# jirsat/wavenets

Measured on AMD Instinct MI355X. Metric: audio samples/sec (training step, 16 kHz mu-law), higher is better.
Workload: dtype f32 (fp16 hi|lo split operands, fp32 accumulate)

## Files before the change

### wavenets_amd/csrc/wn_kernels.h

```cpp
#pragma once
#include "wn_common.h"

struct WnTensorDesc { int64_t off; int64_t len; };

struct WnPrepDesc {
  int64_t src_off;
  int64_t dst_off;
  int32_t I;
  int32_t KK;
  int32_t ld;
  int32_t transpose;
  int32_t q_off;
  int32_t j_off;
  int32_t JT;
  int32_t kind;
};
int wn_launch_prep_table(const WnPrepDesc* d_table, int n, const float* params, float* ws,
                         hipStream_t s, int gx = 16);
int wn_launch_prep_one(WnPrepDesc d, const float* params, float* ws, hipStream_t s);
struct WnVecSumArgs { const float* base; int64_t off0; int64_t stride; int32_t count; int32_t len; float* out; };
int wn_launch_vecsum(WnVecSumArgs a, hipStream_t s);

#define WN_MAXSEG 4
struct WnSeg {
// ... 44 lines not shown
  int32_t act;
  float* y; int32_t ldy;
  int32_t N;
  int32_t B, T;
  float* absmax_out;
  int32_t bwd;
  const float* absmax_in;
  const float* aux; int32_t ld_aux;
  int32_t nshift; int32_t shift[4];
  int32_t cat_loss;
  const int32_t* target;
  float gscale;
  float* loss_rows;
  float* sample_out;
  float inv_lv;
  uint64_t seed, offset;
};
int wn_gemm_planes16s_supported(int N, int plane_k, int nplanes, int ld, int ldy);
int wn_gemm_taps16s_supported(int N, int plane_k, int ntaps, int ld, int ldy);
int wn_launch_gemm_planes16s(const WnGemmPlanesArgs& a, hipStream_t s);

struct WnWgradArgs {
  const float* x; int32_t ldx; int32_t K; int32_t shift;
  const float* g; int32_t ldg; int32_t N;
  int32_t B, T;
  int32_t splits_per_b;
  float* slab;
  float* slab_bias;
};
int wn_wgrad_choose_splits(int B, int T, int K, int N);
int wn_launch_wgrad(const WnWgradArgs& a, hipStream_t s);
struct WnWgJob {
  int64_t x_off, g_off, out_off, bias_off;
  int64_t gmax_off;
  int32_t ldx, ldg, K, N, shift, k0, n0, pad_;
};
struct WnWgLayer {
  int64_t x_off, du_off, z_off, go_off;
  int64_t dwd_off, dbd_off, dwr_off, dbr_off;
  int64_t gmax_u_off, gmax_h_off;
  int32_t dilation, ldz;
};
int wn_wgrad_layer_supported(int R, int D, int KS);
int wn_launch_wgrad_layers(const WnWgLayer* d_layers, int nlayers, int R, float* ws, float* slab, int64_t P, int B,
                           int T, int splits_per_b, hipStream_t s, int inner = 0);
struct WnWgPair {
  int64_t x_off, g_off;
  int64_t w_off, b_off;
  int64_t gmax_off;
  int32_t shift;
  union { int32_t pad_; int32_t nseg; };
  union { int64_t g2_off; int64_t seg_stride; };
  int64_t w2_off, b2_off, gmax2_off;
};
int wn_wgrad_pair_kind(int K, int N);
int wn_launch_wgrad_pairs(int kind, const WnWgPair* d_jobs, int njobs, float* ws, float* slab, int64_t P, int B, int T,
                          int splits_per_b, hipStream_t s);
int wn_wgrad_tr_kind(int K, int N, int taps);
int wn_launch_wgrad_tr(int kind, const WnWgPair* d_jobs, int njobs, float* ws, float* slab, int64_t P, int B, int T,
                       int splits_per_b, hipStream_t s, float* slab2 = nullptr, int64_t P2 = 0);
struct WnBwdPairArgs {
  const float* gu_in;
  const float* gx_res;
  const float* gf;
  const float* ag;
  const float* z; int32_t ldz;
  float* gx_out;
  float* gu_out;
  const float* wx16;
  const float* wu16;
  const float* am_gu_in; const float* am_gf;
  float* am_gx; float* am_gu;
  int32_t B, T, dil;
};
int wn_bwd_pair_supported(int R, int D, int KS, int F0);
int wn_launch_bwd_pair(const WnBwdPairArgs& a, hipStream_t s);
int wn_bwd_s128_supported(int R, int D, int KS, int F0);
int wn_launch_bwd_s128(const WnBwdPairArgs& a, hipStream_t s);
int wn_wgrad_skip_supported(int D, int S, int KZ);
int wn_launch_wgrad_skip(const float* z, int ldz, const float* g, int ldg, int64_t rows, int KZ, int S, int D,
                         int nsplit, float* slab, int64_t P, int64_t w_off0, int64_t w_stride, int64_t b_off0,
                         int64_t b_stride, int nblocks, const float* gmax, hipStream_t s);
int wn_wgrad_tile_k();
int wn_wgrad_tile_n();
int wn_launch_wgrad_batched(const WnWgJob* d_jobs, int njobs, float* ws, float* slab, int64_t P, int B, int T,
                            int splits_per_b, hipStream_t s, bool exact_fp32 = false);
int wn_launch_reduce_table(const float* slab, int nsplit, int64_t P, float* out, const WnTensorDesc* d_table,
                           int n, hipStream_t s, const WnTensorDesc* h_table = nullptr);
struct WnReduceArgs {
  const float* slab; int32_t nsplit; int32_t K; int32_t N;
  float* out; int32_t seg_len; int64_t seg_stride; int32_t accumulate;
  int32_t replicate; int64_t rep_stride;
};
int wn_launch_reduce(const WnReduceArgs& a, hipStream_t s);

struct WnLayerFwdArgs {
  const float* x;
  const float* frag_d;
  const float* frag_r;
  const float* bias_d;
  const float* bias_r;
  const float* cb;
  float* x_out;
  float* o_out;
  float* z_out; int32_t ldz;
  float* ag_out;
// ... 174 lines not shown
```

### wavenets_amd/csrc/wn_train.hip

```cpp
#include "wn_plan_internal.h"

namespace {
using namespace wnp;

void add_jobs(std::vector<WnWgJob>& jobs, int64_t x_off, int ldx, int K, int shift, int64_t g_off, int ldg, int N,
              int64_t out_off, int64_t bias_off, int64_t gmax_off) {
  const int tk = wn_wgrad_tile_k(), tn = wn_wgrad_tile_n();
  for (int k0 = 0; k0 < K; k0 += tk)
    for (int n0 = 0; n0 < N; n0 += tn) {
      WnWgJob j;
      memset(&j, 0, sizeof(j));
      j.x_off = x_off; j.g_off = g_off; j.out_off = out_off; j.bias_off = (k0 == 0) ? bias_off : -1;
      j.gmax_off = gmax_off;
      j.ldx = ldx; j.ldg = ldg; j.K = K; j.N = N; j.shift = shift; j.k0 = k0; j.n0 = n0;
      jobs.push_back(j);
    }
}

int ensure_schedule(const wn_plan* p, wn_exec& e, const WsLayout& L, int B, int T, const TrainPaths& tp) {
  WgSchedule& g = e.wg;
  if (g.valid && g.B == B && g.T == T && g.bsplits == L.bsplits && g.paths == tp) return WN_OK;
  const bool layerk = tp.layerk(), pairk = tp.pairk(), fold = tp.fold;
  std::vector<WnWgLayer> wgl, wgli;
  std::vector<WnWgPair> pairs[3];
// ... 38 lines not shown
      w.dwd_off = p->tensors[c.kernel_t].off; w.dbd_off = p->tensors[c.bias_t].off;
      w.dwr_off = p->tensors[bi.conv1.kernel_t].off; w.dbr_off = p->tensors[bi.conv1.bias_t].off;
      w.gmax_u_off = am_GU(b); w.gmax_h_off = p->S == 0 ? am_skip : am_GH(b + 1);
      w.dilation = c.dil;
      wgl.push_back(w);
    } else if (pairk) {
      const int64_t xoff = tp.drop ? L.XD[b] : L.H[b];
      {
        WnWgPair w;
        memset(&w, 0, sizeof(w));
        w.x_off = xoff; w.g_off = L.GU[b]; w.shift = c.dil;
        w.w_off = p->tensors[c.kernel_t].off;
        w.b_off = p->tensors[c.bias_t].off;
        w.gmax_off = am_GU(b);
        pairs[1].push_back(w);
      }
      WnWgPair w;
      memset(&w, 0, sizeof(w));
      w.x_off = zoff; w.g_off = p->S == 0 ? L.GO[b] : L.GH[b + 1]; w.shift = 0;
      w.w_off = p->tensors[bi.conv1.kernel_t].off; w.b_off = p->tensors[bi.conv1.bias_t].off;
      w.gmax_off = p->S == 0 ? am_skip : am_GH(b + 1);
      w.g2_off = w.w2_off = w.b2_off = w.gmax2_off = -1;
      if (tp.mfused) {
        w.g2_off = L.GF[0]; w.w2_off = (int64_t)b * p->D * p->fold_F0;
        w.b2_off = b == 0 ? (int64_t)p->N * p->D * p->fold_F0 : -1;
        w.gmax2_off = L.absmax + slot.gf(0);
      }
      pairs[2].push_back(w);
    } else {
    for (int i = 0; i < p->LPB; ++i) {
      const ConvInfo& ci = bi.dil[i];
      const bool lastc = i == p->LPB - 1;
      const int64_t xo = i == 0 ? (tp.drop ? L.XD[b] : L.H[b]) : L.P[b][i - 1];
      const int kc = i == 0 ? p->R : p->D, nc = lastc ? 2 * p->D : p->D;
      for (int t = 0; t < p->KS; ++t)
        add_jobs(jobs, xo, kc, kc, (p->KS - 1 - t) * ci.dil, lastc ? L.GU[b] : L.GP[b][i], nc, nc,
                 p->tensors[ci.kernel_t].off + (int64_t)t * kc * nc,
                 t == p->KS - 1 ? p->tensors[ci.bias_t].off : -1, lastc ? am_GU(b) : am_GP(b, i));
      if (!lastc) { cover(ci.kernel_t); cover(ci.bias_t); }
    }
    add_jobs(jobs, zoff, p->Dp, p->D, 0, p->S == 0 ? L.GO[b] : L.GH[b + 1], p->R, p->R,
             p->tensors[bi.conv1.kernel_t].off, p->tensors[bi.conv1.bias_t].off, p->S == 0 ? am_skip : am_GH(b + 1));
    }
    cover(bi.dil.back().kernel_t); cover(bi.dil.back().bias_t);
    cover(bi.conv1.kernel_t); cover(bi.conv1.bias_t);
    if (bi.has_skip && p->c.use_skip && !fold) {
      if (!tp.skipk)
        add_jobs(jobs, zoff, p->Dp, p->D, 0, L.g_skipsum, p->S, p->S,
                 p->tensors[bi.conv_skip.kernel_t].off, p->tensors[bi.conv_skip.bias_t].off, am_skip);
      cover(bi.conv_skip.kernel_t); cover(bi.conv_skip.bias_t);
    }
  }
  if (tp.mtr != 0) {
    const int per = 256 / p->D;
    for (int b0 = 0; b0 < p->N; b0 += per) {
      WnWgPair w;
      memset(&w, 0, sizeof(w));
      w.x_off = L.Z + (int64_t)b0 * B * T * p->Dp;
      w.seg_stride = (int64_t)B * T * p->Dp;
      w.nseg = std::min(per, p->N - b0);
      w.g_off = L.GF[0]; w.shift = 0;
      w.w_off = (int64_t)b0 * p->D * p->fold_F0;
      w.b_off = b0 == 0 ? (int64_t)p->N * p->D * p->fold_F0 : -1;
      w.gmax_off = L.absmax + slot.gf(0);
      w.w2_off = w.b2_off = w.gmax2_off = -1;
      pairs[0].push_back(w);
    }
  }
  const int head_first = (int)jobs.size(), cov_head = (int)cov.size();
  for (size_t i = fold ? 1 : 0; i < p->finals.size(); ++i) {
    const ConvInfo& c = p->finals[i];
    const int64_t xin = (i == 0) ? (p->c.use_skip ? L.skipsum : L.H[p->N]) : L.HA[i - 1];
    if (tp.headpairs() && wn_wgrad_pair_kind(c.cin, c.cout) != 0) {
      WnWgPair w;
      memset(&w, 0, sizeof(w));
      w.x_off = xin; w.g_off = L.GF[i]; w.shift = 0;
      w.w_off = p->tensors[c.kernel_t].off; w.b_off = p->tensors[c.bias_t].off;
      w.gmax_off = L.absmax + slot.gf((int)i);
      const int kind = wn_wgrad_pair_kind(c.cin, c.cout);
      hpairs[kind].push_back(w);
      if (kind == 5) {
        w.g_off += 128; w.w_off += 128; w.b_off += 128;
        hpairs[kind].push_back(w);
      }
    } else {
      add_jobs(jobs, xin, c.cin, c.cin, 0, L.GF[i], c.cout, c.cout, p->tensors[c.kernel_t].off,
               p->tensors[c.bias_t].off, L.absmax + slot.gf((int)i));
    }
    cover(c.kernel_t); cover(c.bias_t);
  }
  std::vector<WnWgPair> all;
  int pfirst[3], hfirst[6] = {0, 0, 0, 0, 0, 0};
  for (int kd = 0; kd <= 2; ++kd) { pfirst[kd] = (int)all.size(); all.insert(all.end(), pairs[kd].begin(), pairs[kd].end()); }
  for (int kd = 1; kd <= 5; ++kd) { hfirst[kd] = (int)all.size(); all.insert(all.end(), hpairs[kd].begin(), hpairs[kd].end()); }
  std::vector<WgSpan> spans;
  auto span = [&](WgSpan::Op op, WgSpan::Slab slab, int kind, int first, size_t count) {
    if (count > 0) spans.push_back(WgSpan{op, slab, kind, first, (int)count});
  };
  const int njobs = (int)jobs.size();
  const bool head_own = tp.head_split && (head_first < njobs || tp.headpairs());
  span(WgSpan::INCONV, WgSpan::BATCH, 0, 0, tp.in_split);
  span(WgSpan::JOBS, WgSpan::BATCH, tp.wg == WG_GENERIC_FP32, 0, head_own ? head_first : njobs);
  if (head_own) span(WgSpan::JOBS, WgSpan::HEAD, 0, head_first, njobs - head_first);
  for (int kd = 1; kd <= 5; ++kd) {
    const int trk = kd == 1 ? 3 : (kd == 3 ? 4 : (kd == 5 ? 5 : (kd == 2 ? 2 : 0)));
    if (trk != 0 && tp.pairk()) span(WgSpan::TR, WgSpan::HEAD, trk, hfirst[kd], hpairs[kd].size());
    else span(WgSpan::PAIRS, WgSpan::HEAD, kd, hfirst[kd], hpairs[kd].size());
  }
  const int n_side = (int)spans.size();
  span(WgSpan::TR, WgSpan::BATCH, 1, pfirst[1], pairs[1].size());
  span(WgSpan::TR, WgSpan::BATCH, tp.mfused ? 6 : 2, pfirst[2], pairs[2].size());
  span(WgSpan::LAYERS, WgSpan::BATCH, 0, 0, wgl.size());
  span(WgSpan::LAYERS, WgSpan::BATCH, 1, 0, wgli.size());
  if (tp.mtr != 0) span(WgSpan::TR, WgSpan::MFOLD, tp.mtr, pfirst[0], pairs[0].size());
  else if (tp.fold) span(WgSpan::SKIP, WgSpan::MFOLD, 0, 0, !tp.mfused);
  else span(WgSpan::SKIP, WgSpan::BATCH, 0, 0, tp.skipk);
  g.valid = false;
  int rc = g.jobs.upload(jobs, 1);
  if (!rc) rc = g.cov.upload(cov);
  if (!rc) rc = g.layers.upload(wgl);
  if (!rc) rc = g.inner.upload(wgli);
  if (!rc) rc = g.pairs.upload(all);
  if (rc) return rc;
  g.h_cov.swap(cov); g.spans.swap(spans);
  g.n_side = n_side; g.overlap = layerk || pairk; g.cov_head = head_own ? cov_head : (int)g.h_cov.size();
  g.B = B; g.T = T; g.bsplits = L.bsplits; g.paths = tp;
  g.valid = true;
  return WN_OK;
}

struct TrainCall {
  wn_exec& e;
  wn_plan* p; const float* params; const float* x_full; const float* cond;
  int B, T, global_batch, n_replicas;
  float* grads; float* loss_out; float* pred_out; float* ws; hipStream_t s;
  WsLayout L;
  int64_t rows;
  float* inputs;
  const float* fragbase; float* slab;
  float* am; AbsmaxSlots slot;
  int nf; float* am_gskip;
  const float* mlast = nullptr;
  TrainPaths tp;
  bool cond_batched = false;
  float* g_x = nullptr; float* g_cond = nullptr;
  int64_t pm = 0;
  float* am_GF(int i) const { return am + slot.gf(i); }
  float* am_GU(int b) const { return am + slot.gu(b); }
  float* am_GH(int b) const { return am + slot.gh(b); }
  float* am_GP(int b, int i) const { return am + slot.gp(b, i); }
  struct Strided { int64_t off, stride; };
  Strided strided(int t0, int t1) const { return {p->tensors[t0].off, p->N > 1 ? p->tensors[t1].off - p->tensors[t0].off : 0}; }
  Strided skip_w{0, 0}, skip_b{0, 0};

  void bind(wn_plan* p_, const float* params_, const float* cond_, int B_, int T_, float* grads_, float* workspace, hipStream_t s_) {
    p = p_; params = params_; x_full = nullptr; cond = cond_; B = B_; T = T_; global_batch = B_; n_replicas = 1;
    grads = grads_; loss_out = nullptr; pred_out = nullptr; ws = workspace; s = s_;
    L = make_layout(p, B, T, true);
    rows = (int64_t)B * T;
    inputs = workspace + L.probs;
    am = workspace + L.absmax;
    nf = (int)p->finals.size();
    slot = AbsmaxSlots{nf, p->N, p->LPB};
    am_gskip = am + slot.gskip();
  }
// ... 185 lines not shown
    rc = wn_launch_sgemm_small(ws + L.mtot, F0, 1, wf0, 1, F0, ws + L.ytmp, p->S, nd1, p->S, F0, s);
    if (rc) return rc;
    const int nzk = (nd1 + 127) / 128;
    if ((int64_t)nzk * p->S * F0 <= L.slab_floats) {
      rc = wn_launch_sgemm_small_batched(ws + L.wsall, 1, p->S, (int64_t)128 * p->S, ws + L.mtot, F0, 1, (int64_t)128 * F0, slab, F0,
                                         (int64_t)p->S * F0, p->S, F0, nd1, nzk, nullptr, 0, s, 128);
      if (rc) return rc;
      WnVecSumArgs v;
      v.base = slab; v.off0 = 0; v.stride = (int64_t)p->S * F0; v.count = nzk; v.len = p->S * F0;
      v.out = grads + p->tensors[c0.kernel_t].off;
      rc = wn_launch_vecsum(v, s);
    } else
    rc = wgrad(ws + L.wsall, p->S, p->S, 0, ws + L.mtot, F0, F0, 1, nd1, grads + p->tensors[c0.kernel_t].off, nullptr, nullptr,
               slab, s);
    if (rc) return rc;
    return wn_launch_skip_scatter(ws + L.ytmp, ws + L.mtot + (int64_t)p->N * p->D * F0, skip_w.off, skip_w.stride, skip_b.off,
                                  skip_b.stride, p->tensors[c0.bias_t].off, p->N, p->D, p->S, F0, grads, s);
  }

  int cond_weight_gradients() {
    int rc;
    const int D2 = 2 * p->D;
    const BlockInfo& b0 = p->blocks[0]; const BlockInfo& b1 = p->blocks[p->N > 1 ? 1 : 0];
    const Strided db = strided(b0.dil.back().bias_t, b1.dil.back().bias_t);
    const Strided cw = strided(b0.conv_cond.kernel_t, b1.conv_cond.kernel_t), cbi = strided(b0.conv_cond.bias_t, b1.conv_cond.bias_t);
    rc = wn_launch_cond_gather(ws + L.bslab, p->nparams, L.bsplits, db.off, db.stride, B, p->N, D2, ws + L.cbt, s);
    if (rc) return rc;
    if (cond_small(p) && (int64_t)p->N * B * p->Cc <= L.slab_floats) {
      rc = wn_launch_sgemm_small_batched(ws + L.cbt, p->N * D2, 1, D2, params + cw.off, 1, D2, cw.stride,
                                         slab, p->Cc, (int64_t)B * p->Cc, B, p->Cc, D2, p->N, nullptr, 0, s);
      if (rc) return rc;
      WnVecSumArgs v;
      v.base = slab; v.off0 = 0; v.stride = (int64_t)B * p->Cc; v.count = p->N; v.len = B * p->Cc; v.out = ws + L.g_m0;
      rc = wn_launch_vecsum(v, s);
    } else
    rc = Gemm(1, B, p->Cc, ceil32(p->Cc)).seg(ws + L.cbt, p->N * D2, p->N * D2, 0, fragbase + p->frag_condB).run(ws + L.g_m0, p->Cc, s);
    if (rc) return rc;
    return wn_launch_cond_wgrad(mlast, ws + L.cbt, B, p->Cc, p->N, D2, grads, cw.off, cw.stride, cbi.off, cbi.stride, s);
  }

  int launch(const WgSpan& sp, hipStream_t st) {
    const WgSchedule& g = e.wg;
    float* out = ws + L.bslab; int64_t pitch = p->nparams; int splits = L.bsplits;
    if (sp.slab == WgSpan::HEAD) { out = ws + L.hslab - L.head_base; pitch = L.head_span; splits = L.hsplits; }
    if (sp.slab == WgSpan::MFOLD) { out = ws + L.mslab; pitch = pm; }
    switch (sp.op) {
      case WgSpan::INCONV:
        return wn_launch_inconv_wgrad(inputs, ws + L.GH[0], B, T, p->R, p->KS, L.isplits, ws + L.islab, (int64_t)(p->KS + 1) * p->R,
                                      0, (int64_t)p->KS * p->R, st);
      case WgSpan::JOBS: return wn_launch_wgrad_batched(g.jobs.d + sp.first, sp.count, ws, out, pitch, B, T, splits, st, sp.kind != 0);
      case WgSpan::PAIRS: return wn_launch_wgrad_pairs(sp.kind, g.pairs.d + sp.first, sp.count, ws, out, pitch, B, T, splits, st);
      case WgSpan::TR:
        return wn_launch_wgrad_tr(sp.kind, g.pairs.d + sp.first, sp.count, ws, out, pitch, B, T, splits, st,
                                  sp.kind == 6 ? ws + L.mslab : nullptr, sp.kind == 6 ? pm : 0);
      case WgSpan::LAYERS: return wn_launch_wgrad_layers(sp.kind ? g.inner.d : g.layers.d, sp.count, p->R, ws, out, pitch, B, T, splits, st, sp.kind);
      case WgSpan::SKIP:
        if (sp.slab == WgSpan::MFOLD)
          return wn_launch_wgrad_skip(ws + L.Z, p->Dp, ws + L.GF[0], p->fold_F0, rows, p->N * p->D, p->fold_F0, p->D, B * splits, out, pitch,
                                      0, (int64_t)p->D * p->fold_F0, (int64_t)p->N * p->D * p->fold_F0, 0, 1, am_GF(0), st);
        return wn_launch_wgrad_skip(ws + L.Z, p->Dp, ws + L.g_skipsum, p->S, rows, p->N * p->D, p->S, p->D, B * splits, out, pitch,
                                    skip_w.off, skip_w.stride, skip_b.off, skip_b.stride, p->N, am_gskip, st);
    }
    return WN_E_INVALID;
  }

  int weight_gradients() {
    int rc;
    const WgSchedule& g = e.wg;
    if (e.phase_on) (void)hipEventRecord(e.phase_ev[3], s);
    const bool fork = g.overlap && wn_debug_get(9) != 1;
    if (fork && !e.side) {
      WN_HIP_CHECK(hipStreamCreateWithFlags(&e.side, hipStreamNonBlocking));
      WN_HIP_CHECK(hipEventCreateWithFlags(&e.ev_fork, hipEventDisableTiming));
      WN_HIP_CHECK(hipEventCreateWithFlags(&e.ev_join, hipEventDisableTiming));
    }
    struct SideJoin {
      wn_exec& e; hipStream_t s; bool armed;
      ~SideJoin() {
        if (!armed) return;
        if (hipEventRecord(e.ev_join, e.side) != hipSuccess || hipStreamWaitEvent(s, e.ev_join, 0) != hipSuccess)
          (void)hipStreamSynchronize(e.side);
      }
    } side_join{e, s, false};
    if (fork) {
      WN_HIP_CHECK(hipEventRecord(e.ev_fork, s));
      WN_HIP_CHECK(hipStreamWaitEvent(e.side, e.ev_fork, 0));
      side_join.armed = true;
    }
    size_t i = 0;
    for (; i < (size_t)g.n_side; ++i)
      if ((rc = launch(g.spans[i], fork ? e.side : s))) return rc;
    if (fork) WN_HIP_CHECK(hipEventRecord(e.ev_join, e.side));
    for (; i < g.spans.size(); ++i)
      if ((rc = launch(g.spans[i], s))) return rc;
    if (tp.fold && (rc = fold_weight_gradients())) return rc;
    if (fork) { WN_HIP_CHECK(hipStreamWaitEvent(s, e.ev_join, 0)); side_join.armed = false; }
    if (cond_batched && (rc = cond_weight_gradients())) return rc;
    const int cov0 = tp.in_split ? 2 : 0, ncov = (int)g.h_cov.size(), cov1 = g.cov_head;
    rc = wn_launch_reduce_table(ws + L.bslab, B * L.bsplits, p->nparams, grads, g.cov.d + cov0, cov1 - cov0, s, g.h_cov.data() + cov0);
    if (rc) return rc;
    if (tp.in_split && (rc = wn_launch_reduce_table(ws + L.islab, B * L.isplits, (int64_t)(p->KS + 1) * p->R, grads, g.cov.d, 2, s, g.h_cov.data())))
      return rc;
    if (cov1 < ncov && (rc = wn_launch_reduce_table(ws + L.hslab - L.head_base, B * L.hsplits, L.head_span, grads, g.cov.d + cov1, ncov - cov1,
                                                    s, g.h_cov.data() + cov1)))
      return rc;
    if (!p->c.use_skip && p->S > 0) {
      for (const BlockInfo& bi : p->blocks) {
        rc = wn_launch_fill(grads + p->tensors[bi.conv_skip.kernel_t].off, 0.f, p->tensors[bi.conv_skip.kernel_t].len, s);
// ... 195 lines not shown
```

### wavenets_amd/csrc/wn_wgrad_layer.hip

```cpp
#include "wn_split16.h"

using namespace wn_split16;

template <int C32, bool INNER>
__global__ __launch_bounds__(256, 2) void wn_wgrad_layer_kernel(const WnWgLayer* layers, float* ws, float* slab,
                                                                int64_t P, int B, int T, int spb) {
  constexpr int R = 32 * C32, NCH = INNER ? 3 * R : 6 * R;
  constexpr int DUW = INNER ? R : 2 * R;
  constexpr int NXU = INNER ? 2 * 2 * R : 2 * 4 * R;
  constexpr int NU = 1 + (NXU + 255) / 256;
  constexpr int PLANE = NCH * 32;
  constexpr int STAGE = 2 * PLANE;
  constexpr int NJ = INNER ? C32 : ((C32 == 2) ? 4 : 1);
  __shared__ __attribute__((aligned(16))) unsigned char smem[2 * STAGE + 2 * NCH * 4];
  float* bpart = reinterpret_cast<float*>(smem + 2 * STAGE);
  const int tid = threadIdx.x, lane = tid & 63, wave = tid >> 6;
  const int tl = lane & 31, h = lane >> 5;
  const WnWgLayer Ld = layers[blockIdx.y];
  const int split = blockIdx.x;
  const int ub = split / spb, sp = split % spb;
  int len = (T + spb - 1) / spb;
  len = (len + 15) & ~15;
  const int r0 = sp * len, r1 = min(T, r0 + len);
  const int d = Ld.dilation;

  const float* const gmax_u = Ld.gmax_u_off >= 0 ? ws + Ld.gmax_u_off : nullptr;
  const float* const gmax_h = Ld.gmax_h_off >= 0 ? ws + Ld.gmax_h_off : nullptr;
  float su = 1.0f, inv_u = 1.0f, sh = 1.0f, inv_h = 1.0f;
  if (gmax_u) pow2_scale(*gmax_u, su, inv_u);
  if (gmax_h) pow2_scale(*gmax_h, sh, inv_h);

  const float* uptr[NU];
  int ushift[NU], uch[NU], uhh[NU];
  float uscale[NU];
  bool uvalid[NU], ugrad[NU];
  {
    uvalid[0] = tid < 2 * DUW;
    const int c = uvalid[0] ? tid % DUW : 0;
    uch[0] = 2 * R + c;
    uhh[0] = uvalid[0] ? tid / DUW : 0;
    ushift[0] = 0;
    uscale[0] = su;
    ugrad[0] = true;
    uptr[0] = ws + Ld.du_off + (int64_t)ub * T * DUW + c;
  }
#pragma unroll
  for (int i = 1; i < NU; ++i) {
    const int uid = (i - 1) * 256 + tid;
    uvalid[i] = uid < NXU;
    const int c = uvalid[i] ? uid % (NXU / 2) : 0;
    uhh[i] = uvalid[i] ? uid / (NXU / 2) : 0;
    ushift[i] = 0;
    uscale[i] = 1.0f;
    ugrad[i] = false;
    if (c < 2 * R) {
      uch[i] = c;
      uptr[i] = ws + Ld.x_off + (int64_t)ub * T * R + (c % R);
      ushift[i] = c < R ? d : 0;
    } else if (c < 3 * R) {
      uch[i] = 4 * R + (c - 2 * R);
      uptr[i] = ws + Ld.z_off + (int64_t)ub * T * R + (c - 2 * R);
    } else {
      uch[i] = 5 * R + (c - 3 * R);
      uptr[i] = ws + Ld.go_off + (int64_t)ub * T * R + (c - 3 * R);
      uscale[i] = sh;
      ugrad[i] = true;
    }
  }
  float bsum[NU];
#pragma unroll
  for (int i = 0; i < NU; ++i) bsum[i] = 0.f;

  auto load_chunk = [&](int t0, float (&v)[NU][8]) {
    const bool interior = (t0 + 16 <= r1) && (t0 - d >= 0);
    wn_static_for<NU>([&](auto ic) {
      constexpr int i = decltype(ic)::value;
      constexpr int LD = (i == 0) ? DUW : R;
      const int tb = t0 + 8 * uhh[i] - ushift[i];
      const float* p = uptr[i] + (int64_t)tb * LD;
      if (interior && uvalid[i]) {
#pragma unroll
        for (int e = 0; e < 8; ++e) v[i][e] = p[e * LD];
      } else {
#pragma unroll
        for (int e = 0; e < 8; ++e) {
          const bool ok = uvalid[i] && (t0 + 8 * uhh[i] + e < r1) && (tb + e >= 0);
          v[i][e] = ok ? p[e * LD] : 0.f;
        }
      }
    });
  };
  auto store_chunk = [&](int stage, const float (&v)[NU][8]) {
    unsigned char* st = smem + stage * STAGE;
#pragma unroll
    for (int i = 0; i < NU; ++i) {
      if (!uvalid[i]) continue;
      h8 hi, lo;
      float s8 = 0.f;
#pragma unroll
      for (int e = 0; e < 8; ++e) s8 += v[i][e];
      split8s(v[i], uscale[i], hi, lo);
      if (ugrad[i]) bsum[i] += s8;
      *reinterpret_cast<h8*>(st + uch[i] * 32 + uhh[i] * 16) = hi;
      *reinterpret_cast<h8*>(st + PLANE + uch[i] * 32 + uhh[i] * 16) = lo;
    }
  };

  const int xt = (C32 == 2) ? wave : (wave >> 1);
  const int j0 = (C32 == 2 || INNER) ? 0 : (wave & 1);
  const bool has_d = !INNER || C32 == 2 || (wave & 1) == 0;
  const bool has_r = !INNER && ((C32 == 2) || wave == 0);
  const int zt = (C32 == 2) ? (wave >> 1) : 0, gt = (C32 == 2) ? (wave & 1) : 0;
  f32x16 acc[NJ], accr;
#pragma unroll
  for (int j = 0; j < NJ; ++j)
#pragma unroll
    for (int r = 0; r < 16; ++r) acc[j][r] = 0.f;
#pragma unroll
  for (int r = 0; r < 16; ++r) accr[r] = 0.f;

  auto compute = [&](int stage) {
    const unsigned char* st = smem + stage * STAGE + tl * 32 + h * 16;
    auto frag = [&](int cb, h8& hi, h8& lo) {
      hi = *reinterpret_cast<const h8*>(st + cb * 32);
      lo = *reinterpret_cast<const h8*>(st + PLANE + cb * 32);
    };
    h8 ah, al;
    if (has_d) frag(32 * xt, ah, al);
#pragma unroll
    for (int j = 0; j < NJ; ++j) {
      if (!has_d) break;
      h8 bh, bl;
      frag(2 * R + 32 * (j0 + j), bh, bl);
      mfma3(ah, al, bh, bl, acc[j]);
    }
    if (has_r) {
      h8 zh, zl, gh, gl;
      frag(4 * R + 32 * zt, zh, zl);
      frag(5 * R + 32 * gt, gh, gl);
      mfma3(zh, zl, gh, gl, accr);
    }
  };

  float va[NU][8], vb[NU][8];
  if (r0 < r1) {
    load_chunk(r0, va);
    if (r0 + 16 < r1) load_chunk(r0 + 16, vb);
    store_chunk(0, va);
  }
  __syncthreads();
  int stage = 0;
  for (int t0 = r0; t0 < r1; t0 += 32) {
    if (t0 + 32 < r1) load_chunk(t0 + 32, va);
    compute(stage);
    if (t0 + 16 < r1) store_chunk(stage ^ 1, vb);
    __syncthreads();
    if (t0 + 16 >= r1) break;
    if (t0 + 48 < r1) load_chunk(t0 + 48, vb);
    compute(stage ^ 1);
    if (t0 + 32 < r1) store_chunk(stage, va);
    __syncthreads();
  }

  float* row = slab + (int64_t)split * P;
  {
    const int tap = xt / C32, kt = xt % C32;
#pragma unroll
    for (int j = 0; j < NJ; ++j)
#pragma unroll
      for (int r = 0; r < 16; ++r) {
        const int k = 32 * kt + wn_drow(r, h);
        if (has_d) row[Ld.dwd_off + ((int64_t)tap * R + k) * DUW + 32 * (j0 + j) + tl] = acc[j][r] * inv_u;
      }
    if (has_r) {
#pragma unroll
      for (int r = 0; r < 16; ++r) {
        const int k = 32 * zt + wn_drow(r, h);
        row[Ld.dwr_off + (int64_t)k * R + 32 * gt + tl] = accr[r] * inv_h;
      }
    }
  }
#pragma unroll
  for (int i = 0; i < NU; ++i)
    if (uvalid[i] && ugrad[i]) bpart[uhh[i] * NCH + uch[i]] = bsum[i];
  __syncthreads();
  for (int c = tid; c < NCH; c += 256) {
    if (c >= 2 * R && c < 2 * R + DUW) { if (Ld.dbd_off >= 0) row[Ld.dbd_off + (c - 2 * R)] = bpart[c] + bpart[NCH + c]; }
    else if (!INNER && c >= 5 * R) row[Ld.dbr_off + (c - 5 * R)] = bpart[c] + bpart[NCH + c];
  }
}

int wn_wgrad_layer_supported(int R, int D, int KS) { return R == D && (R == 32 || R == 64) && KS == 2; }

int wn_launch_wgrad_layers(const WnWgLayer* d_layers, int nlayers, int R, float* ws, float* slab, int64_t P, int B,
                           int T, int splits_per_b, hipStream_t s, int inner) {
  if (nlayers <= 0) return WN_OK;
  const dim3 grid((unsigned)(B * splits_per_b), (unsigned)nlayers);
  if (R == 64 && inner) hipLaunchKernelGGL((wn_wgrad_layer_kernel<2, true>), grid, dim3(256), 0, s, d_layers, ws, slab, P, B, T, splits_per_b);
  else if (R == 32 && inner) hipLaunchKernelGGL((wn_wgrad_layer_kernel<1, true>), grid, dim3(256), 0, s, d_layers, ws, slab, P, B, T, splits_per_b);
  else if (R == 64) hipLaunchKernelGGL((wn_wgrad_layer_kernel<2, false>), grid, dim3(256), 0, s, d_layers, ws, slab, P, B, T, splits_per_b);
  else if (R == 32) hipLaunchKernelGGL((wn_wgrad_layer_kernel<1, false>), grid, dim3(256), 0, s, d_layers, ws, slab, P, B, T, splits_per_b);
  else { wn_set_error("wgrad_layers: unsupported width %d", R); return WN_E_UNSUPPORTED; }
  WN_HIP_CHECK(hipGetLastError());
  return WN_OK;
}
```

### wavenets_amd/csrc/wn_wgrad_tr.hip

```cpp
#include "wn_split16.h"

using namespace wn_split16;

typedef short wt_s4 __attribute__((ext_vector_type(4)));

namespace {

constexpr int WT_ROWS = 32;

template <int PITCH>
__device__ __forceinline__ h8 wt_frag(const unsigned char* lanebase, int off) {
  const wt_s4 a = __builtin_amdgcn_ds_read_tr16_b64_v4i16((__attribute__((address_space(3))) wt_s4*)(lanebase + off));
  const wt_s4 b = __builtin_amdgcn_ds_read_tr16_b64_v4i16((__attribute__((address_space(3))) wt_s4*)(lanebase + off + 4 * PITCH));
  h8 r;
  const h4 ha = *reinterpret_cast<const h4*>(&a), hb = *reinterpret_cast<const h4*>(&b);
  r[0] = ha[0]; r[1] = ha[1]; r[2] = ha[2]; r[3] = ha[3]; r[4] = hb[0]; r[5] = hb[1]; r[6] = hb[2]; r[7] = hb[3];
  return r;
}

}

template <int KC, int NC, int TAPS, int LDX, int LDG, int LDW, int TKW, int TNW, bool G2 = false, int XSEG = 0>
__global__ __launch_bounds__(512, 2) void wn_wgrad_tr_kernel(const WnWgPair* jobs, float* ws, float* slab, int64_t P, int B,
                                                             int T, int spb, float* slab2, int64_t P2) {
  constexpr int XC = TAPS * KC, NCH = XC + NC;
  constexpr int PITCH = NCH * 2 + 64;
  constexpr int PLANE = WT_ROWS * PITCH, STAGE = 2 * PLANE;
  constexpr int KT = XC / 32, NT = NC / 32;
  static_assert((KT / TKW) * (NT / TNW) == 8 && KT % TKW == 0 && NT % TNW == 0, "8 waves tile the output block");
  static_assert((PITCH / 4) % 64 == 16, "row pitch must rotate the banks by a quarter");
  static_assert(XSEG == 0 || (TAPS == 1 && !G2 && LDX == XSEG && KC % XSEG == 0 && XSEG % 32 == 0), "segmented X");
  constexpr int XPR = KC / 4, GPR = NC / 4;
  constexpr int XRP = 512 / XPR, GRP = 512 / GPR;
  constexpr int XP = WT_ROWS / XRP, GP = WT_ROWS / GRP;
  __shared__ __attribute__((aligned(16))) unsigned char smem[2 * STAGE];
  static_assert(2 * STAGE <= 160 * 1024 && GRP * NC * 4 <= 2 * STAGE, "LDS");
  const int tid = threadIdx.x, lane = tid & 63, wave = __builtin_amdgcn_readfirstlane(tid >> 6);
  const int tl = lane & 31, h = lane >> 5;
  const WnWgPair J = jobs[blockIdx.y];
  const int split = blockIdx.x;
  const int ub = split / spb, sp = split % spb;
  int len = (T + spb - 1) / spb;
  len = (len + WT_ROWS - 1) & ~(WT_ROWS - 1);
  const int r0 = sp * len, r1 = min(T, r0 + len);
  const int d = J.shift;

  float gsc = 1.0f, inv = 1.0f, gsc2 = 1.0f, inv2 = 1.0f;
  if (J.gmax_off >= 0) pow2_scale(ws[J.gmax_off], gsc, inv);
  if constexpr (G2) if (J.gmax2_off >= 0) pow2_scale(ws[J.gmax2_off], gsc2, inv2);

  const int xr = tid / XPR, xc = (tid % XPR) * 4;
  const int gr = tid / GPR, gc = (tid % GPR) * 4;
  const int nseg = XSEG > 0 ? J.nseg : 0;
  const bool xvalid = XSEG == 0 || xc / (XSEG > 0 ? XSEG : 1) < nseg;
  const float* xbase = XSEG > 0 ? ws + J.x_off + (int64_t)(xvalid ? xc / (XSEG > 0 ? XSEG : 1) : 0) * J.seg_stride + (int64_t)ub * T * LDX + xc % (XSEG > 0 ? XSEG : 1)
                                : ws + J.x_off + (int64_t)ub * T * LDX + xc;
  const bool upper = G2 && gc >= NC / 2;
  const float* gbase = upper ? ws + J.g2_off + (int64_t)ub * T * LDG + (gc - NC / 2) : ws + J.g_off + (int64_t)ub * T * LDG + gc;
  const float gs_t = upper ? gsc2 : gsc;
  struct Regs { f32x4 xs[TAPS][XP]; f32x4 gv[GP]; };
  Regs ra, rb;
  float bsum[4] = {0.f, 0.f, 0.f, 0.f};
  const f32x4 zero4 = {0.f, 0.f, 0.f, 0.f};

  auto load = [&](int t0, Regs& q) {
    f32x4 (&xs)[TAPS][XP] = q.xs;
    f32x4 (&gv)[GP] = q.gv;
#pragma unroll
    for (int k = 0; k < XP; ++k) {
      const int t = t0 + xr + XRP * k;
      const int tc = min(t, T - 1);
      if (XSEG > 0) {
        xs[0][k] = ldg4(xbase + (int64_t)tc * LDX);
      } else {
        xs[0][k] = ldg4(xbase + (int64_t)max(tc - d, 0) * LDX);
        if constexpr (TAPS == 2) xs[1][k] = ldg4(xbase + (int64_t)tc * LDX);
      }
    }
#pragma unroll
    for (int k = 0; k < GP; ++k) {
      const int t = min(t0 + gr + GRP * k, T - 1);
      gv[k] = ldg4(gbase + (int64_t)t * LDG);
    }
  };
  auto store = [&](int stage, const Regs& q, int t0) {
    const f32x4 (&xs)[TAPS][XP] = q.xs;
    const f32x4 (&gv)[GP] = q.gv;
    unsigned char* st = smem + stage * STAGE;
    const bool interior = (t0 + WT_ROWS <= r1) && (t0 - d >= 0);
#pragma unroll
    for (int k = 0; k < XP; ++k) {
      unsigned char* row = st + (xr + XRP * k) * PITCH;
      const int t = t0 + xr + XRP * k;
#pragma unroll
      for (int tp = 0; tp < TAPS; ++tp) {
        h4 hi, lo;
        const bool ok = interior || (t < r1 && (XSEG > 0 || (TAPS == 2 && tp == TAPS - 1) || t - d >= 0));
        const f32x4 xv = (ok && xvalid) ? xs[tp][k] : zero4;
        split4s(xv, 1.0f, hi, lo);
        *reinterpret_cast<h4*>(row + (tp * KC + xc) * 2) = hi;
        *reinterpret_cast<h4*>(row + PLANE + (tp * KC + xc) * 2) = lo;
      }
    }
#pragma unroll
    for (int k = 0; k < GP; ++k) {
      h4 hi, lo;
      unsigned char* row = st + (gr + GRP * k) * PITCH;
      const f32x4 g4 = (interior || t0 + gr + GRP * k < r1) ? gv[k] : zero4;
      split4s(g4, gs_t, hi, lo);
      bsum[0] += g4.x; bsum[1] += g4.y; bsum[2] += g4.z; bsum[3] += g4.w;
      *reinterpret_cast<h4*>(row + (XC + gc) * 2) = hi;
      *reinterpret_cast<h4*>(row + PLANE + (XC + gc) * 2) = lo;
    }
  };

  constexpr int WKD = KT / TKW;
  const int kt0 = TKW * (wave % WKD), nt0 = TNW * (wave / WKD);
  f32x16 acc[TKW][TNW];
#pragma unroll
  for (int i = 0; i < TKW; ++i)
#pragma unroll
    for (int j = 0; j < TNW; ++j)
#pragma unroll
      for (int r = 0; r < 16; ++r) acc[i][j][r] = 0.f;
  const int lb = (8 * h + ((lane & 15) >> 2)) * PITCH + (16 * ((lane >> 4) & 1) + 4 * (lane & 3)) * 2;
  auto compute = [&](int stage) {
    const unsigned char* base = smem + stage * STAGE + lb;
    wn_static_for<2>([&](auto kc) {
      constexpr int ks = decltype(kc)::value;
      constexpr int ro = ks * 16 * PITCH;
      h8 ah[TKW], al[TKW];
#pragma unroll
      for (int i = 0; i < TKW; ++i) {
        ah[i] = wt_frag<PITCH>(base, ro + 32 * (kt0 + i) * 2);
        al[i] = wt_frag<PITCH>(base, ro + PLANE + 32 * (kt0 + i) * 2);
      }
#pragma unroll
      for (int j = 0; j < TNW; ++j) {
        const h8 bh = wt_frag<PITCH>(base, ro + (XC + 32 * (nt0 + j)) * 2);
        const h8 bl = wt_frag<PITCH>(base, ro + PLANE + (XC + 32 * (nt0 + j)) * 2);
#pragma unroll
        for (int i = 0; i < TKW; ++i) {
          mfma3(ah[i], al[i], bh, bl, acc[i][j]);
        }
      }
    });
  };

  constexpr bool DEEP = TAPS == 1;
  if constexpr (DEEP) {
    load(r0, ra);
    load(r0 + WT_ROWS, rb);
    store(0, ra, r0);
    load(r0 + 2 * WT_ROWS, ra);
    __syncthreads();
    for (int t0 = r0; t0 < r1; t0 += 2 * WT_ROWS) {
      store(1, rb, t0 + WT_ROWS);
      load(t0 + 3 * WT_ROWS, rb);
      compute(0);
      __syncthreads();
      if (t0 + WT_ROWS >= r1) break;
      store(0, ra, t0 + 2 * WT_ROWS);
      load(t0 + 4 * WT_ROWS, ra);
      compute(1);
      __syncthreads();
    }
  } else {
    load(r0, ra);
    store(0, ra, r0);
    load(r0 + WT_ROWS, ra);
    __syncthreads();
    int st = 0;
    for (int t0 = r0; t0 < r1; t0 += WT_ROWS, st ^= 1) {
      store(st ^ 1, ra, t0 + WT_ROWS);
      load(t0 + 2 * WT_ROWS, ra);
      compute(st);
      __syncthreads();
    }
  }

  float* row = slab + (int64_t)split * P;
  float* row2 = G2 ? slab2 + (int64_t)split * P2 : nullptr;
#pragma unroll
  for (int i = 0; i < TKW; ++i) {
    if (XSEG > 0 && 32 * (kt0 + i) >= nseg * XSEG) continue;
#pragma unroll
    for (int j = 0; j < TNW; ++j) {
      const int nt = nt0 + j;
      const bool up = G2 && nt >= NT / 2;
      float* tbase = (up ? row2 + J.w2_off + 32 * (nt - NT / 2) : row + J.w_off + 32 * nt) + (int64_t)(32 * (kt0 + i)) * LDW + tl;
      const float iv = up ? inv2 : inv;
#pragma unroll
      for (int r = 0; r < 16; ++r) tbase[wn_drow(r, h) * LDW] = acc[i][j][r] * iv;
    }
  }
  if (J.b_off >= 0 || (G2 && J.b2_off >= 0)) {
    float* bpart = reinterpret_cast<float*>(smem);
#pragma unroll
    for (int e = 0; e < 4; ++e) bpart[gr * NC + gc + e] = bsum[e];
    __syncthreads();
    for (int n = tid; n < NC; n += 512) {
      float s8 = 0.f;
#pragma unroll
      for (int g = 0; g < GRP; ++g) s8 += bpart[g * NC + n];
      if (G2 && n >= NC / 2) { if (J.b2_off >= 0) row2[J.b2_off + n - NC / 2] = s8; }
      else if (J.b_off >= 0) row[J.b_off + n] = s8;
    }
  }
}

int wn_wgrad_tr_kind(int K, int N, int taps) {
  if (taps == 2) return (K == 128 && N == 256) ? 1 : 0;
  if (K == 128 && N == 128) return 2;
  if (K == 128 && N == 256) return 3;
  if (K == 256 && N == 128) return 4;
  if (K == 256 && N == 256) return 5;
  return 0;
}

int wn_launch_wgrad_tr(int kind, const WnWgPair* d_jobs, int njobs, float* ws, float* slab, int64_t P, int B, int T,
                       int splits_per_b, hipStream_t s, float* slab2, int64_t P2) {
  if (njobs <= 0) return WN_OK;
  const dim3 grid((unsigned)(B * splits_per_b), (unsigned)njobs);
#define WT_LAUNCH(...) hipLaunchKernelGGL((wn_wgrad_tr_kernel<__VA_ARGS__>), grid, dim3(512), 0, s, d_jobs, ws, slab, P, B, T, splits_per_b, slab2, P2)
  switch (kind) {
    case 1: WT_LAUNCH(128, 256, 2, 128, 256, 256, 2, 4); break;
    case 2: WT_LAUNCH(128, 128, 1, 128, 128, 128, 1, 2); break;
    case 3: WT_LAUNCH(128, 256, 1, 128, 256, 256, 1, 4); break;
    case 4: WT_LAUNCH(256, 128, 1, 256, 128, 128, 2, 2); break;
    case 5: WT_LAUNCH(256, 128, 1, 256, 256, 256, 2, 2); break;
    case 6:
      if (!slab2) { wn_set_error("wgrad_tr: kind 6 needs the second slab"); return WN_E_INVALID; }
      WT_LAUNCH(128, 256, 1, 128, 128, 128, 1, 4, true);
      break;
    case 7: WT_LAUNCH(256, 128, 1, 64, 128, 128, 2, 2, false, 64); break;
    case 8: WT_LAUNCH(256, 128, 1, 32, 128, 128, 2, 2, false, 32); break;
    default: wn_set_error("wgrad_tr: unknown kind %d", kind); return WN_E_UNSUPPORTED;
  }
#undef WT_LAUNCH
  WN_HIP_CHECK(hipGetLastError());
  return WN_OK;
}
```

Measured before the change: 22.82 million.

## Fuse per-layer 1x1 conv weight grad into the folded skip wgrad kernel

For mtr kind 7, the folded-skip transposed wgrad kernel now also loads each layer's g_h gradient segment alongside z and computes that layer's 1x1 conv1 weight and bias gradients. Z is then read once for both products instead of again in the per-layer kernel. The layer kernel gets a NO1X1 variant that drops the 1x1 part. Segments per job drop from 256/D to 2, so each z tile is loaded once, at the cost of more jobs, extra LDS for an fp32 staging buffer, and an extra MFMA accumulator per wave.

```diff
diff --git a/wavenets_amd/csrc/wn_kernels.h b/wavenets_amd/csrc/wn_kernels.h
--- a/wavenets_amd/csrc/wn_kernels.h
+++ b/wavenets_amd/csrc/wn_kernels.h
@@ -120,6 +120,7 @@
   union { int32_t pad_; int32_t nseg; };
   union { int64_t g2_off; int64_t seg_stride; };
   int64_t w2_off, b2_off, gmax2_off;
+  struct Seg { int64_t g_off, gmax_off, w_off, b_off; } seg[2];
 };
 int wn_wgrad_pair_kind(int K, int N);
 int wn_launch_wgrad_pairs(int kind, const WnWgPair* d_jobs, int njobs, float* ws, float* slab, int64_t P, int B, int T,
diff --git a/wavenets_amd/csrc/wn_train.hip b/wavenets_amd/csrc/wn_train.hip
--- a/wavenets_amd/csrc/wn_train.hip
+++ b/wavenets_amd/csrc/wn_train.hip
@@ -114,7 +114,8 @@
     }
   }
   if (tp.mtr != 0) {
-    const int per = 256 / p->D;
+    const bool zonce = tp.mtr == 7;
+    const int per = zonce ? 2 : 256 / p->D;
     for (int b0 = 0; b0 < p->N; b0 += per) {
       WnWgPair w;
       memset(&w, 0, sizeof(w));
@@ -126,6 +127,12 @@
       w.b_off = b0 == 0 ? (int64_t)p->N * p->D * p->fold_F0 : -1;
       w.gmax_off = L.absmax + slot.gf(0);
       w.w2_off = w.b2_off = w.gmax2_off = -1;
+      for (int sg = 0; zonce && sg < 2; ++sg) {
+        const int b = b0 + (sg < w.nseg ? sg : 0);
+        const BlockInfo& bi = p->blocks[b];
+        w.seg[sg].g_off = L.GH[b + 1]; w.seg[sg].gmax_off = am_GH(b + 1);
+        w.seg[sg].w_off = p->tensors[bi.conv1.kernel_t].off; w.seg[sg].b_off = p->tensors[bi.conv1.bias_t].off;
+      }
       pairs[0].push_back(w);
     }
   }
@@ -172,7 +179,7 @@
   const int n_side = (int)spans.size();
   span(WgSpan::TR, WgSpan::BATCH, 1, pfirst[1], pairs[1].size());
   span(WgSpan::TR, WgSpan::BATCH, tp.mfused ? 6 : 2, pfirst[2], pairs[2].size());
-  span(WgSpan::LAYERS, WgSpan::BATCH, 0, 0, wgl.size());
+  span(WgSpan::LAYERS, WgSpan::BATCH, tp.mtr == 7 ? 2 : 0, 0, wgl.size());
   span(WgSpan::LAYERS, WgSpan::BATCH, 1, 0, wgli.size());
   if (tp.mtr != 0) span(WgSpan::TR, WgSpan::MFOLD, tp.mtr, pfirst[0], pairs[0].size());
   else if (tp.fold) span(WgSpan::SKIP, WgSpan::MFOLD, 0, 0, !tp.mfused);
@@ -464,8 +471,9 @@
       case WgSpan::PAIRS: return wn_launch_wgrad_pairs(sp.kind, g.pairs.d + sp.first, sp.count, ws, out, pitch, B, T, splits, st);
       case WgSpan::TR:
         return wn_launch_wgrad_tr(sp.kind, g.pairs.d + sp.first, sp.count, ws, out, pitch, B, T, splits, st,
-                                  sp.kind == 6 ? ws + L.mslab : nullptr, sp.kind == 6 ? pm : 0);
-      case WgSpan::LAYERS: return wn_launch_wgrad_layers(sp.kind ? g.inner.d : g.layers.d, sp.count, p->R, ws, out, pitch, B, T, splits, st, sp.kind);
+                                  sp.kind == 6 ? ws + L.mslab : (sp.kind == 7 ? ws + L.bslab : nullptr),
+                                  sp.kind == 6 ? pm : (sp.kind == 7 ? p->nparams : 0));
+      case WgSpan::LAYERS: return wn_launch_wgrad_layers(sp.kind == 1 ? g.inner.d : g.layers.d, sp.count, p->R, ws, out, pitch, B, T, splits, st, sp.kind);
       case WgSpan::SKIP:
         if (sp.slab == WgSpan::MFOLD)
           return wn_launch_wgrad_skip(ws + L.Z, p->Dp, ws + L.GF[0], p->fold_F0, rows, p->N * p->D, p->fold_F0, p->D, B * splits, out, pitch,
diff --git a/wavenets_amd/csrc/wn_wgrad_layer.hip b/wavenets_amd/csrc/wn_wgrad_layer.hip
--- a/wavenets_amd/csrc/wn_wgrad_layer.hip
+++ b/wavenets_amd/csrc/wn_wgrad_layer.hip
@@ -2,12 +2,14 @@
 
 using namespace wn_split16;
 
-template <int C32, bool INNER>
+template <int C32, bool INNER, bool NO1X1 = false>
 __global__ __launch_bounds__(256, 2) void wn_wgrad_layer_kernel(const WnWgLayer* layers, float* ws, float* slab,
                                                                 int64_t P, int B, int T, int spb) {
-  constexpr int R = 32 * C32, NCH = INNER ? 3 * R : 6 * R;
+  static_assert(!(INNER && NO1X1), "INNER has no 1x1 part already");
+  constexpr bool ONE = !INNER && !NO1X1;
+  constexpr int R = 32 * C32, NCH = INNER ? 3 * R : (NO1X1 ? 4 * R : 6 * R);
   constexpr int DUW = INNER ? R : 2 * R;
-  constexpr int NXU = INNER ? 2 * 2 * R : 2 * 4 * R;
+  constexpr int NXU = ONE ? 2 * 4 * R : 2 * 2 * R;
   constexpr int NU = 1 + (NXU + 255) / 256;
   constexpr int PLANE = NCH * 32;
   constexpr int STAGE = 2 * PLANE;
@@ -109,7 +111,7 @@
   const int xt = (C32 == 2) ? wave : (wave >> 1);
   const int j0 = (C32 == 2 || INNER) ? 0 : (wave & 1);
   const bool has_d = !INNER || C32 == 2 || (wave & 1) == 0;
-  const bool has_r = !INNER && ((C32 == 2) || wave == 0);
+  const bool has_r = ONE && ((C32 == 2) || wave == 0);
   const int zt = (C32 == 2) ? (wave >> 1) : 0, gt = (C32 == 2) ? (wave & 1) : 0;
   f32x16 acc[NJ], accr;
 #pragma unroll
@@ -186,7 +188,7 @@
   __syncthreads();
   for (int c = tid; c < NCH; c += 256) {
     if (c >= 2 * R && c < 2 * R + DUW) { if (Ld.dbd_off >= 0) row[Ld.dbd_off + (c - 2 * R)] = bpart[c] + bpart[NCH + c]; }
-    else if (!INNER && c >= 5 * R) row[Ld.dbr_off + (c - 5 * R)] = bpart[c] + bpart[NCH + c];
+    else if (ONE && c >= 5 * R) row[Ld.dbr_off + (c - 5 * R)] = bpart[c] + bpart[NCH + c];
   }
 }
 
@@ -196,7 +198,9 @@
                            int T, int splits_per_b, hipStream_t s, int inner) {
   if (nlayers <= 0) return WN_OK;
   const dim3 grid((unsigned)(B * splits_per_b), (unsigned)nlayers);
-  if (R == 64 && inner) hipLaunchKernelGGL((wn_wgrad_layer_kernel<2, true>), grid, dim3(256), 0, s, d_layers, ws, slab, P, B, T, splits_per_b);
+  if (R == 64 && inner == 2) hipLaunchKernelGGL((wn_wgrad_layer_kernel<2, false, true>), grid, dim3(256), 0, s, d_layers, ws, slab, P, B, T, splits_per_b);
+  else if (inner == 2) { wn_set_error("wgrad_layers: no form without the 1x1 part at width %d", R); return WN_E_UNSUPPORTED; }
+  else if (R == 64 && inner) hipLaunchKernelGGL((wn_wgrad_layer_kernel<2, true>), grid, dim3(256), 0, s, d_layers, ws, slab, P, B, T, splits_per_b);
   else if (R == 32 && inner) hipLaunchKernelGGL((wn_wgrad_layer_kernel<1, true>), grid, dim3(256), 0, s, d_layers, ws, slab, P, B, T, splits_per_b);
   else if (R == 64) hipLaunchKernelGGL((wn_wgrad_layer_kernel<2, false>), grid, dim3(256), 0, s, d_layers, ws, slab, P, B, T, splits_per_b);
   else if (R == 32) hipLaunchKernelGGL((wn_wgrad_layer_kernel<1, false>), grid, dim3(256), 0, s, d_layers, ws, slab, P, B, T, splits_per_b);
diff --git a/wavenets_amd/csrc/wn_wgrad_tr.hip b/wavenets_amd/csrc/wn_wgrad_tr.hip
--- a/wavenets_amd/csrc/wn_wgrad_tr.hip
+++ b/wavenets_amd/csrc/wn_wgrad_tr.hip
@@ -20,24 +20,27 @@
 
 }
 
-template <int KC, int NC, int TAPS, int LDX, int LDG, int LDW, int TKW, int TNW, bool G2 = false, int XSEG = 0>
+template <int KC, int NC, int TAPS, int LDX, int LDG, int LDW, int TKW, int TNW, bool G2 = false, int XSEG = 0, bool GSEG = false>
 __global__ __launch_bounds__(512, 2) void wn_wgrad_tr_kernel(const WnWgPair* jobs, float* ws, float* slab, int64_t P, int B,
                                                              int T, int spb, float* slab2, int64_t P2) {
-  constexpr int XC = TAPS * KC, NCH = XC + NC;
+  constexpr int XC = TAPS * KC, GC0 = XC + (GSEG ? KC : 0), NCH = GC0 + NC;
   constexpr int PITCH = NCH * 2 + 64;
   constexpr int PLANE = WT_ROWS * PITCH, STAGE = 2 * PLANE;
   constexpr int KT = XC / 32, NT = NC / 32;
   static_assert((KT / TKW) * (NT / TNW) == 8 && KT % TKW == 0 && NT % TNW == 0, "8 waves tile the output block");
   static_assert((PITCH / 4) % 64 == 16, "row pitch must rotate the banks by a quarter");
   static_assert(XSEG == 0 || (TAPS == 1 && !G2 && LDX == XSEG && KC % XSEG == 0 && XSEG % 32 == 0), "segmented X");
+  static_assert(!GSEG || (XSEG > 0 && KC == 2 * XSEG && TKW == 1 && NT / TNW == XSEG / 32), "one g_o tile per wave");
   constexpr int XPR = KC / 4, GPR = NC / 4;
   constexpr int XRP = 512 / XPR, GRP = 512 / GPR;
   constexpr int XP = WT_ROWS / XRP, GP = WT_ROWS / GRP;
-  __shared__ __attribute__((aligned(16))) unsigned char smem[2 * STAGE];
-  static_assert(2 * STAGE <= 160 * 1024 && GRP * NC * 4 <= 2 * STAGE, "LDS");
+  constexpr int FBS = GSEG ? WT_ROWS * KC * 4 : 0;
+  __shared__ __attribute__((aligned(16))) unsigned char smem[2 * STAGE + 2 * FBS];
+  static_assert(2 * STAGE + 2 * FBS <= 160 * 1024 && (GRP * NC + (GSEG ? 2 * KC : 0)) * 4 <= 2 * STAGE, "LDS");
   const int tid = threadIdx.x, lane = tid & 63, wave = __builtin_amdgcn_readfirstlane(tid >> 6);
   const int tl = lane & 31, h = lane >> 5;
   const WnWgPair J = jobs[blockIdx.y];
+  const WnWgPair::Seg* const segs = jobs[blockIdx.y].seg;
   const int split = blockIdx.x;
   const int ub = split / spb, sp = split % spb;
   int len = (T + spb - 1) / spb;
@@ -58,9 +61,17 @@
   const bool upper = G2 && gc >= NC / 2;
   const float* gbase = upper ? ws + J.g2_off + (int64_t)ub * T * LDG + (gc - NC / 2) : ws + J.g_off + (int64_t)ub * T * LDG + gc;
   const float gs_t = upper ? gsc2 : gsc;
-  struct Regs { f32x4 xs[TAPS][XP]; f32x4 gv[GP]; };
+  const int hseg = (GSEG && xvalid) ? xc / (XSEG > 0 ? XSEG : 1) : 0;
+  const float* hbase = GSEG ? ws + segs[hseg].g_off + (int64_t)ub * T * XSEG + xc % (XSEG > 0 ? XSEG : 1) : nullptr;
+  float hs_t = 1.0f;
+  if constexpr (GSEG) {
+    float unused;
+    if (segs[hseg].gmax_off >= 0) pow2_scale(ws[segs[hseg].gmax_off], hs_t, unused);
+  }
+  struct Regs { f32x4 xs[TAPS][XP]; f32x4 gv[GP]; f32x4 hv[GSEG ? XP : 1]; };
   Regs ra, rb;
   float bsum[4] = {0.f, 0.f, 0.f, 0.f};
+  float hsum = 0.f;
   const f32x4 zero4 = {0.f, 0.f, 0.f, 0.f};
 
   auto load = [&](int t0, Regs& q) {
@@ -72,6 +83,7 @@
       const int tc = min(t, T - 1);
       if (XSEG > 0) {
         xs[0][k] = ldg4(xbase + (int64_t)tc * LDX);
+        if constexpr (GSEG) q.hv[k] = ldg4(hbase + (int64_t)tc * XSEG);
       } else {
         xs[0][k] = ldg4(xbase + (int64_t)max(tc - d, 0) * LDX);
         if constexpr (TAPS == 2) xs[1][k] = ldg4(xbase + (int64_t)tc * LDX);
@@ -101,6 +113,14 @@
         *reinterpret_cast<h4*>(row + (tp * KC + xc) * 2) = hi;
         *reinterpret_cast<h4*>(row + PLANE + (tp * KC + xc) * 2) = lo;
       }
+      if constexpr (GSEG) {
+        h4 hi, lo;
+        const f32x4 g4 = ((interior || t < r1) && xvalid) ? q.hv[k] : zero4;
+        split4s(g4, hs_t, hi, lo);
+        *reinterpret_cast<f32x4*>(smem + 2 * STAGE + stage * FBS + ((xr + XRP * k) * KC + xc) * 4) = g4;
+        *reinterpret_cast<h4*>(row + (XC + xc) * 2) = hi;
+        *reinterpret_cast<h4*>(row + PLANE + (XC + xc) * 2) = lo;
+      }
     }
 #pragma unroll
     for (int k = 0; k < GP; ++k) {
@@ -109,8 +129,8 @@
       const f32x4 g4 = (interior || t0 + gr + GRP * k < r1) ? gv[k] : zero4;
       split4s(g4, gs_t, hi, lo);
       bsum[0] += g4.x; bsum[1] += g4.y; bsum[2] += g4.z; bsum[3] += g4.w;
-      *reinterpret_cast<h4*>(row + (XC + gc) * 2) = hi;
-      *reinterpret_cast<h4*>(row + PLANE + (XC + gc) * 2) = lo;
+      *reinterpret_cast<h4*>(row + (GC0 + gc) * 2) = hi;
+      *reinterpret_cast<h4*>(row + PLANE + (GC0 + gc) * 2) = lo;
     }
   };
 
@@ -123,9 +143,26 @@
     for (int j = 0; j < TNW; ++j)
 #pragma unroll
       for (int r = 0; r < 16; ++r) acc[i][j][r] = 0.f;
+  const int wseg = GSEG ? 32 * kt0 / (XSEG > 0 ? XSEG : 1) : 0;
+  const int ht = wave / WKD;
+  f32x16 accr;
+#pragma unroll
+  for (int r = 0; r < 16; ++r) accr[r] = 0.f;
   const int lb = (8 * h + ((lane & 15) >> 2)) * PITCH + (16 * ((lane >> 4) & 1) + 4 * (lane & 3)) * 2;
   auto compute = [&](int stage) {
     const unsigned char* base = smem + stage * STAGE + lb;
+    if constexpr (GSEG) {
+      if (wave < 2 * KC / 64) {
+        const float* fb = reinterpret_cast<const float*>(smem + 2 * STAGE + stage * FBS) + (8 * (tid / KC)) * KC + tid % KC;
+#pragma unroll
+        for (int c16 = 0; c16 < WT_ROWS / 16; ++c16) {
+          float s8 = 0.f;
+#pragma unroll
+          for (int e = 0; e < 8; ++e) s8 += fb[(16 * c16 + e) * KC];
+          hsum += s8;
+        }
+      }
+    }
     wn_static_for<2>([&](auto kc) {
       constexpr int ks = decltype(kc)::value;
       constexpr int ro = ks * 16 * PITCH;
@@ -137,12 +174,17 @@
       }
 #pragma unroll
       for (int j = 0; j < TNW; ++j) {
-        const h8 bh = wt_frag<PITCH>(base, ro + (XC + 32 * (nt0 + j)) * 2);
-        const h8 bl = wt_frag<PITCH>(base, ro + PLANE + (XC + 32 * (nt0 + j)) * 2);
+        const h8 bh = wt_frag<PITCH>(base, ro + (GC0 + 32 * (nt0 + j)) * 2);
+        const h8 bl = wt_frag<PITCH>(base, ro + PLANE + (GC0 + 32 * (nt0 + j)) * 2);
 #pragma unroll
         for (int i = 0; i < TKW; ++i) {
           mfma3(ah[i], al[i], bh, bl, acc[i][j]);
         }
+      }
+      if constexpr (GSEG) {
+        const h8 bh = wt_frag<PITCH>(base, ro + (XC + XSEG * wseg + 32 * ht) * 2);
+        const h8 bl = wt_frag<PITCH>(base, ro + PLANE + (XC + XSEG * wseg + 32 * ht) * 2);
+        mfma3(ah[0], al[0], bh, bl, accr);
       }
     });
   };
@@ -194,6 +236,23 @@
       for (int r = 0; r < 16; ++r) tbase[wn_drow(r, h) * LDW] = acc[i][j][r] * iv;
     }
   }
+  if constexpr (GSEG) {
+    if (wseg < nseg) {
+      float sc, iv = 1.0f;
+      if (segs[wseg].gmax_off >= 0) pow2_scale(ws[segs[wseg].gmax_off], sc, iv);
+      float* tbase = slab2 + (int64_t)split * P2 + segs[wseg].w_off + (int64_t)(32 * kt0 - XSEG * wseg) * XSEG + 32 * ht + tl;
+#pragma unroll
+      for (int r = 0; r < 16; ++r) tbase[wn_drow(r, h) * XSEG] = accr[r] * iv;
+    }
+    float* hpart = reinterpret_cast<float*>(smem) + GRP * NC;
+    if (tid < 2 * KC) hpart[tid] = hsum;
+    __syncthreads();
+    for (int n = tid; n < KC; n += 512) {
+      const int sg = n / (XSEG > 0 ? XSEG : 1);
+      if (sg >= nseg || segs[sg].b_off < 0) continue;
+      slab2[(int64_t)split * P2 + segs[sg].b_off + n % (XSEG > 0 ? XSEG : 1)] = hpart[n] + hpart[KC + n];
+    }
+  }
   if (J.b_off >= 0 || (G2 && J.b2_off >= 0)) {
     float* bpart = reinterpret_cast<float*>(smem);
 #pragma unroll
@@ -233,7 +292,10 @@
       if (!slab2) { wn_set_error("wgrad_tr: kind 6 needs the second slab"); return WN_E_INVALID; }
       WT_LAUNCH(128, 256, 1, 128, 128, 128, 1, 4, true);
       break;
-    case 7: WT_LAUNCH(256, 128, 1, 64, 128, 128, 2, 2, false, 64); break;
+    case 7:
+      if (!slab2) { wn_set_error("wgrad_tr: kind 7 needs the second slab"); return WN_E_INVALID; }
+      WT_LAUNCH(128, 128, 1, 64, 128, 128, 1, 2, false, 64, true);
+      break;
     case 8: WT_LAUNCH(256, 128, 1, 32, 128, 128, 2, 2, false, 32); break;
     default: wn_set_error("wgrad_tr: unknown kind %d", kind); return WN_E_UNSUPPORTED;
   }
```

Result: faster. 23.42 million, median of 6 (+2.6%).
